# XuanHuang0/VANeRF

Hardware: AMD Instinct MI355X
Metric: rendered rays/sec (64 samples/ray) + PSNR vs ref, 512x334 view (higher is better)
Workload: dtype bf16x3 (bf16 MFMA on hi+lo split operands, f32 accumulate; per-sample outputs within 3.3e-5 of the f32 kernel); 1 GPU; configs/vanerf.json eval view 512x334, 64 coarse + 64 importance samples/ray, two-hand mesh 1558 verts / 3108 faces, 1 source view 256x256, random trained-like weights; rays=171008, parallelism=single

## Files before the change

include/vanerf_hip.h:

```cpp
#ifndef VANERF_HIP_H
#define VANERF_HIP_H

#include <stdint.h>

#ifdef __cplusplus
extern "C" {
#endif

#define VANERF_ABI_VERSION 12

#define VANERF_OK 0
#define VANERF_EINVAL (-22)
#define VANERF_ENOMEM (-12)
#define VANERF_EHIP (-5)

#define VANERF_NV 1558
#define VANERF_NV_HAND 779
#define VANERF_NKPT 42
#define VANERF_PE_LEVELS 3

typedef struct {
    const float* geo_at0_w1;
    const float* geo_at0_w2;
    const float* geo_ated0_w1;
// ... 73 lines not shown
    const float* sphere;
    const float* tnorm;
    const int32_t* orig;
    const float* cbox;
    int nfp, nc;
    const int32_t* cell_start;
    const int32_t* cell_tri;
    const float* cell_rec;
    const float* grid;
    const float* vsort;
    const float* vbox;
    int nvc;
    const float* cdisc;
} VanerfMeshAccel;

int64_t vanerf_mesh_accel_bytes(int nv, int nf, int G, int cell_capacity);
int vanerf_mesh_accel_build(const float* verts, int nv, const int32_t* faces, int nf, int G, int cell_capacity, void* tables,
                            int64_t tables_bytes, VanerfMeshAccel* out, void* stream);

int vanerf_mesh_query_accel(const VanerfMeshAccel* accel, const float* verts, int nv, const int32_t* faces, int nf,
                            const float* vert_vis, const float* pts, int64_t n, float* sdf, uint8_t* vis, int32_t* face,
                            int32_t* knn_idx, int grid_nx, int grid_ny, int grid_s, void* queue_word, void* stream);

int vanerf_knn1(const float* verts4, int nv, const float* pts, int64_t n, int32_t* idx, void* stream);

int vanerf_query_samples(const VanerfWeights* w, const VanerfFrame* frame, const float* pts, const float* query_sdf,
                         const uint8_t* query_vis, const int32_t* knn_idx, const float* noise, const int32_t* order, int raw, int64_t n,
                         float* out, uint8_t* valid, void* queue_word , const float* vertex_products,
                         void* stream);

int vanerf_vertex_products(const VanerfWeights* w, const VanerfFrame* frame, float* table, int64_t cap_floats, void* stream);

int vanerf_query_order(const VanerfFrame* frame, const float* pts, int64_t n, int32_t* order, void* scratch, int64_t scratch_bytes,
                       void* stream);
int64_t vanerf_query_order_scratch(int64_t n);

int vanerf_composite(const float* rgba, const float* z, const float* mesh_sdf, int Sa, const float* rgba_n, const float* mesh_sdf_n, int Sn,
                     const int32_t* src, int R, float beta, float* color, float* depth, float* alpha, float* sdf, float* contrib, void* stream);
int vanerf_composite_handle(const VanerfWeights* w, const float* rgba, const float* z, const float* mesh_sdf, int Sa, const float* rgba_n,
                            const float* mesh_sdf_n, int Sn, const int32_t* src, int R, float* color, float* depth, float* alpha, float* sdf,
                            float* contrib, void* stream);
int vanerf_eval_func(const float* raw_a, const uint8_t* valid_a, const float* raw_b, const uint8_t* valid_b, const int32_t* src, const float* noise,
                     int Sa, int Sb, int R, float invalid_sdf, float* rgba_a, float* rgba_b, void* stream);
int vanerf_composite_backward(const VanerfWeights* w, const float* rgba, const float* z, const float* mesh_sdf, int Sa, const float* rgba_n,
                              const float* mesh_sdf_n, int Sn, const int32_t* src, int R, const float* g_color, const float* g_depth,
                              const float* g_alpha, const float* g_sdf, float* d_rgba, float* d_rgba_n, float* d_beta, void* stream);
// ... 120 lines not shown
```

vanerf_amd/_ffi.py:

```python
import ctypes
import os

import torch
from ctypes import POINTER, Structure, c_char_p, c_double, c_float, c_int, c_int64, c_uint, c_uint64, c_void_p

_HERE = os.path.dirname(os.path.abspath(__file__))
LIB_PATH = os.environ.get("VANERF_HIP_LIB") or os.path.join(_HERE, "lib", "libvanerf_hip.so")
ABI_VERSION = 12
NUM_LAYERS = 20

if not os.path.exists(LIB_PATH):
    raise ImportError(f"{LIB_PATH} not found: the HIP extension is required (run `python -m vanerf_amd.build`)")
lib = ctypes.CDLL(LIB_PATH)

_FP = c_void_p


class VanerfWeightTable(Structure):
    _fields_ = [
        ("geo_at0_w1", _FP), ("geo_at0_w2", _FP), ("geo_ated0_w1", _FP), ("geo_ated0_w2", _FP),
        ("geo_at1_w1", _FP), ("geo_at1_w2", _FP), ("geo_ated1_w1", _FP), ("geo_ated1_w2", _FP),
        ("l1_v", _FP * 3), ("l1_g", _FP * 3), ("l1_b", _FP * 3), ("l1_w3", _FP), ("l1_b3", _FP),
        ("l2_v", _FP * 2), ("l2_g", _FP * 2), ("l2_b", _FP * 2), ("l2_w2", _FP), ("l2_b2", _FP),
        ("ibr_w", _FP), ("ibr_b", _FP),
# ... 34 lines not shown
    _fields_ = [("index", _FP), ("hit", _FP), ("z", _FP), ("color", _FP), ("depth", _FP), ("alpha", _FP), ("color_fine", _FP), ("depth_fine", _FP),
                ("alpha_fine", _FP), ("sdf", _FP), ("z_fine", _FP)]


_SIGS = {
    "vanerf_abi_version": (c_int, []),
    "vanerf_last_error": (c_char_p, []),
    "vanerf_mesh_cluster_size": (c_int, []),
    "vanerf_mesh_accel_bytes": (c_int64, [c_int, c_int, c_int, c_int]),
    "vanerf_mesh_accel_build": (c_int, [_FP, c_int, _FP, c_int, c_int, c_int, c_void_p, c_int64, POINTER(VanerfMeshAccel), c_void_p]),
    "vanerf_weights_pack": (c_int, [POINTER(VanerfWeightTable), c_int, POINTER(c_void_p)]),
    "vanerf_weights_free": (c_int, [c_void_p]),
    "vanerf_weights_update": (c_int, [c_void_p, POINTER(VanerfWeightTable), _FP, c_void_p]),
    "vanerf_weights_short_groups": (c_int, [c_void_p, POINTER(c_uint64)]),
    "vanerf_weights_pack_host": (c_int, [POINTER(VanerfWeightTable), _FP, c_int64, POINTER(c_int64), POINTER(c_uint)]),
    "vanerf_weights_stream_host": (c_int, [POINTER(VanerfWeightTable), c_int, _FP, c_int64, POINTER(c_int64)]),
    "vanerf_weights_download": (c_int, [c_void_p, c_int, _FP, c_int64, POINTER(c_int64)]),
    "vanerf_ray_setup": (c_int, [POINTER(VanerfPassDesc), _FP, _FP, _FP, _FP, _FP, _FP, _FP, c_void_p]),
    "vanerf_sample_points": (c_int, [_FP, _FP, _FP, c_int, c_int, c_int, _FP, c_void_p]),
    "vanerf_vertex_visibility": (c_int, [_FP, _FP, c_int, _FP, c_int, c_int, _FP, _FP, c_void_p]),
    "vanerf_mesh_query": (c_int, [_FP, c_int, _FP, c_int, _FP, _FP, c_int64, _FP, _FP, _FP, c_void_p]),
    "vanerf_mesh_query_accel": (c_int, [POINTER(VanerfMeshAccel), _FP, c_int, _FP, c_int, _FP, _FP, c_int64, _FP, _FP, _FP, _FP, c_int, c_int, c_int,
                                        _FP, c_void_p]),
    "vanerf_knn1": (c_int, [_FP, c_int, _FP, c_int64, _FP, c_void_p]),
    "vanerf_query_samples": (c_int, [c_void_p, POINTER(VanerfFrame), _FP, _FP, _FP, _FP, _FP, _FP, c_int, c_int64, _FP, _FP, _FP, _FP, c_void_p]),
    "vanerf_vertex_products": (c_int, [c_void_p, POINTER(VanerfFrame), _FP, c_int64, c_void_p]),
    "vanerf_query_forward_spill": (c_int, [c_void_p, POINTER(VanerfFrame), _FP, _FP, _FP, _FP, c_int64, c_int64, _FP, _FP, _FP, _FP, _FP, c_void_p]),
    "vanerf_query_backward": (c_int, [c_void_p, _FP, _FP, _FP, _FP, _FP, _FP, c_int64, c_int64, _FP, _FP, _FP, _FP, c_void_p]),
    "vanerf_weight_products": (c_int, [_FP, _FP, c_int64, c_int, c_int, _FP, c_void_p]),
    "vanerf_weight_products_size": (c_int, [POINTER(c_int64)]),
    "vanerf_spill_rows": (c_int, [POINTER(c_int), POINTER(c_int), POINTER(c_int), POINTER(c_int)]),
    "vanerf_layer_slots": (c_int, [c_int, _FP, c_int]),
    "vanerf_layer_rows": (c_int, [c_int, POINTER(c_int), POINTER(c_int), POINTER(c_int)]),
    "vanerf_query_order": (c_int, [POINTER(VanerfFrame), _FP, c_int64, _FP, _FP, c_int64, c_void_p]),
    "vanerf_query_order_scratch": (c_int64, [c_int64]),
    "vanerf_composite": (c_int, [_FP, _FP, _FP, c_int, _FP, _FP, c_int, _FP, c_int, c_float, _FP, _FP, _FP, _FP, _FP, c_void_p]),
    "vanerf_eval_func": (c_int, [_FP, _FP, _FP, _FP, _FP, _FP, c_int, c_int, c_int, c_float, _FP, _FP, c_void_p]),
    "vanerf_composite_handle": (c_int, [c_void_p, _FP, _FP, _FP, c_int, _FP, _FP, c_int, _FP, c_int, _FP, _FP, _FP, _FP, _FP, c_void_p]),
    "vanerf_composite_backward": (c_int, [c_void_p, _FP, _FP, _FP, c_int, _FP, _FP, c_int, _FP, c_int, _FP, _FP, _FP, _FP, _FP, _FP, _FP, c_void_p]),
    "vanerf_importance_merge": (c_int, [_FP, _FP, _FP, _FP, c_int, c_int, c_int, _FP, _FP, _FP, _FP, c_void_p]),
    "vanerf_importance_sample": (c_int, [_FP, _FP, _FP, _FP, c_int, c_int, c_int, _FP, _FP, c_void_p]),
    "vanerf_render_pass_scratch": (c_int64, [c_int, c_int, c_int, c_int, c_int, c_int]),
    "vanerf_render_pass": (c_int, [c_void_p, POINTER(VanerfFrame), POINTER(VanerfMeshAccel), _FP, c_int, _FP, c_int, POINTER(VanerfPassDesc),
                                   POINTER(VanerfPassOut), _FP, c_int64, _FP, c_void_p]),
    "vanerf_scatter_add_rows": (c_int, [_FP, _FP, _FP, c_int64, c_int64, c_int, _FP, c_int, c_void_p]),
    "vanerf_bilinear_taps": (c_int, [_FP, c_int64, c_int, c_int, _FP, _FP, c_void_p]),
# ... 46 lines not shown
```

vanerf_amd/csrc/mesh_kernels.hip:

```cpp
#include "common.h"

using namespace vanerf;

namespace {

struct f3 { float x, y, z; };
__device__ __forceinline__ f3 sub3(f3 a, f3 b) { return {a.x - b.x, a.y - b.y, a.z - b.z}; }
__device__ __forceinline__ float dot3(f3 a, f3 b) { return (a.x * b.x + a.y * b.y) + a.z * b.z; }
__device__ __forceinline__ f3 madd3(f3 a, f3 d, float t) { return {a.x + d.x * t, a.y + d.y * t, a.z + d.z * t}; }

__device__ __forceinline__ float point_tri_dist2_q(f3 p, f3 a, f3 b, f3 c, f3& q)
{
    const f3 ab = sub3(b, a), ac = sub3(c, a), ap = sub3(p, a);
    const float d1 = dot3(ab, ap), d2 = dot3(ac, ap);
    if (d1 <= 0.0f && d2 <= 0.0f) {
        q = a;
    } else {
        const f3 bp = sub3(p, b);
        const float d3 = dot3(ab, bp), d4 = dot3(ac, bp);
        if (d3 >= 0.0f && d4 <= d3) {
            q = b;
        } else {
            const float vc = d1 * d4 - d3 * d2;
            if (vc <= 0.0f && d1 >= 0.0f && d3 <= 0.0f) {
// ... 281 lines not shown
    v = OP(v, DPP<0x142, 0xA>(v));                                                                        \
    v = OP(v, DPP<0x143, 0xC>(v));
__device__ __forceinline__ float wave_min_f(float v) { VANERF_WAVE_REDUCE(float, dpp_f, fminf) return __int_as_float(__builtin_amdgcn_readlane(__float_as_int(v), 63)); }
__device__ __forceinline__ float wave_max_f(float v) { VANERF_WAVE_REDUCE(float, dpp_f, fmaxf) return __int_as_float(__builtin_amdgcn_readlane(__float_as_int(v), 63)); }
__device__ __forceinline__ int wave_min_i(int v) { VANERF_WAVE_REDUCE(int, dpp_i, min) return __builtin_amdgcn_readlane(v, 63); }
#undef VANERF_WAVE_REDUCE

__device__ __forceinline__ float uni(float v) { return __int_as_float(__builtin_amdgcn_readfirstlane(__float_as_int(v))); }

__device__ __forceinline__ float box_dist2(f3 p, const float* b)
{
    const float dx = fmaxf(fmaxf(b[0] - p.x, p.x - b[3]), 0.0f);
    const float dy = fmaxf(fmaxf(b[1] - p.y, p.y - b[4]), 0.0f);
    const float dz = fmaxf(fmaxf(b[2] - p.z, p.z - b[5]), 0.0f);
    return (dx * dx + dy * dy) + dz * dz;
}

template <int ND>
__global__ __launch_bounds__(MA_BLOCK) void mesh_query_accel_kernel(const VanerfMeshAccel A, const float* __restrict__ V,
                                                                    const int32_t* __restrict__ F, const float* __restrict__ vert_vis,
                                                                    const float* __restrict__ P, long long n, float* __restrict__ sdf,
                                                                    uint8_t* __restrict__ vis, int32_t* __restrict__ face,
                                                                    int32_t* __restrict__ knn, int gnx, int gny, int gS,
                                                                    unsigned long long* __restrict__ queue)
{
    extern __shared__ float4 s_dyn[];
    __shared__ unsigned short s_list[MA_BLOCK / 64][TL_LIST];
    __shared__ __attribute__((aligned(16))) float s_cand[MA_BLOCK / 64][TL_CAND][12];
    __shared__ float s_dit[MA_BLOCK / 64][TL_IT][64];
    float4* s_vs = s_dyn;
    float* s_vbox = reinterpret_cast<float*>(s_vs + A.nvc * CL);
    float* s_box = s_vbox + A.nvc * 6;
    for (int k = threadIdx.x; k < A.nc * 6; k += MA_BLOCK) s_box[k] = A.cbox[k];
    for (int k = threadIdx.x; k < A.nvc * 6; k += MA_BLOCK) s_vbox[k] = A.vbox[k];
    for (int k = threadIdx.x; k < A.nvc * CL; k += MA_BLOCK) s_vs[k] = reinterpret_cast<const float4*>(A.vsort)[k];
    const float grid_y0 = A.grid[0], grid_z0 = A.grid[1], grid_cy = A.grid[2], grid_cz = A.grid[3];
    const int grid_G = __float_as_int(A.grid[4]);
    __syncthreads();
    const int lane = threadIdx.x & 63;
    auto lane_now = [&]() { int l = lane; asm volatile("" : "+v"(l)); return l; };
    auto claim = [&]() {
        unsigned long long v = 0ull;
        if (lane == 0) v = atomicAdd(queue, 1ull);
        return (long long)(((unsigned long long)(unsigned)__builtin_amdgcn_readfirstlane((int)(v >> 32)) << 32) |
                           (unsigned)__builtin_amdgcn_readfirstlane((int)v));
    };
    const int ntx = (gnx + 7) >> 3, nty = (gny + 7) >> 3;
    const int gD = (gS + ND - 1) / ND;
    const long long nwork = gnx > 0 ? (long long)ntx * nty * gD : (n + 64 * ND - 1) / (64 * ND);
#ifdef VANERF_MESH_PHASES
    unsigned long long ph[16] = {}, tprev = __builtin_amdgcn_s_memtime();
#endif
    for (long long w = claim(); w < nwork; w = claim()) {
        int item_d0 = 0, item_x0 = 0, item_y0 = 0;
        if (gnx > 0) {
            const unsigned wu = (unsigned)w, tile = wu / (unsigned)gD;
            item_d0 = __builtin_amdgcn_readfirstlane((int)(wu % (unsigned)gD) * ND);
            item_x0 = __builtin_amdgcn_readfirstlane((int)(tile % (unsigned)ntx) * 8);
            item_y0 = __builtin_amdgcn_readfirstlane((int)(tile / (unsigned)ntx) * 8);
        }
        auto locate = [&](int k, bool& act) -> long long {
            long long i;
            if (gnx > 0) {
                const int d = item_d0 + k;
                const int l = lane_now();
                const int rx = item_x0 + (l & 7), ry = item_y0 + (l >> 3);
                act = rx < gnx && ry < gny && d < gS;
                i = ((long long)min(ry, gny - 1) * gnx + min(rx, gnx - 1)) * gS + min(d, gS - 1);
            } else {
                i = (w * ND + k) * 64 + lane;
                act = i < n;
                i = act ? i : n - 1;
            }
            return i;
        };
        f3 pk[ND];
#pragma unroll
        for (int k = 0; k < ND; ++k) {
            bool act;
            const long long i = locate(k, act);
            pk[k] = {P[3 * i], P[3 * i + 1], P[3 * i + 2]};
        }
        MPH(0);
        float tlo[3] = {pk[0].x, pk[0].y, pk[0].z}, thi[3] = {pk[0].x, pk[0].y, pk[0].z};
#pragma unroll
        for (int k = 1; k < ND; ++k) {
// ... 592 lines not shown
        if (n == 0) return;
        if (!verts || !faces || !vert_vis || !pts || !sdf || !vis) throw_error("vanerf_mesh_query: null argument");
        if (nv <= 0 || nf <= 0 || n < 0) throw_error("vanerf_mesh_query: nv=%d nf=%d n=%lld", nv, nf, (long long)n);
        if (n == 0) return;
        hipLaunchKernelGGL(mesh_query_kernel, dim3((unsigned)((n + MQ_BLOCK - 1) / MQ_BLOCK)), dim3(MQ_BLOCK), 0, (hipStream_t)stream,
                           verts, faces, nf, vert_vis, pts, (long long)n, sdf, vis, face);
        HIP_CHECK(hipGetLastError());
    });
}

extern "C" int vanerf_knn1(const float* verts4, int nv, const float* pts, int64_t n, int32_t* idx, void* stream)
{
    return guarded([&] {
        if (n == 0) return;
        if (!verts4 || !pts || !idx) throw_error("vanerf_knn1: null argument");
        if (nv <= 0 || nv > 8192 || n < 0) throw_error("vanerf_knn1: nv=%d n=%lld", nv, (long long)n);
        if (n == 0) return;
        hipLaunchKernelGGL(knn1_kernel, dim3((unsigned)((n + 255) / 256)), dim3(256), sizeof(float4) * nv, (hipStream_t)stream,
                           reinterpret_cast<const float4*>(verts4), nv, pts, (long long)n, idx);
        HIP_CHECK(hipGetLastError());
    });
}

extern "C" int vanerf_mesh_query_accel(const VanerfMeshAccel* accel, const float* verts, int nv, const int32_t* faces, int nf,
                                       const float* vert_vis, const float* pts, int64_t n, float* sdf, uint8_t* vis, int32_t* face,
                                       int32_t* knn_idx, int grid_nx, int grid_ny, int grid_s, void* queue_word, void* stream)
{
    return guarded([&] {
        if (n == 0) return;
        if (!accel || !verts || !faces || !vert_vis || !pts || !sdf || !vis) throw_error("vanerf_mesh_query_accel: null argument");
        const VanerfMeshAccel& A = *accel;
        if (!A.tri || !A.sphere || !A.tnorm || !A.orig || !A.cbox || !A.cdisc || !A.cell_start || !A.cell_tri || !A.cell_rec || !A.grid) throw_error("vanerf_mesh_query_accel: accel has a null pointer");
        if (A.nc <= 0 || A.nc > MA_MAX_CLUSTERS || A.nfp != A.nc * CL || A.nfp < nf) throw_error("vanerf_mesh_query_accel: bad cluster table (nc=%d nfp=%d nf=%d)", A.nc, A.nfp, nf);
        if (nv <= 0 || nf <= 0 || n < 0) throw_error("vanerf_mesh_query_accel: nv=%d nf=%d n=%lld", nv, nf, (long long)n);
        if (!A.vsort || !A.vbox || A.nvc <= 0 || A.nvc > MA_MAX_VCLUSTERS || A.nvc * CL < nv)
            throw_error("vanerf_mesh_query_accel: bad vertex cluster table (nvc=%d nv=%d)", A.nvc, nv);
        const size_t lds = sizeof(float) * ((size_t)A.nvc * CL * 4 + (size_t)A.nvc * 6 + (size_t)A.nc * 6);
        if (lds > 140 * 1024) throw_error("vanerf_mesh_query_accel: mesh too large for the LDS-resident tables (%zu bytes)", lds);
        if (lds > 64 * 1024) {
            HIP_CHECK(hipFuncSetAttribute(reinterpret_cast<const void*>(mesh_query_accel_kernel<1>), hipFuncAttributeMaxDynamicSharedMemorySize, (int)lds));
            HIP_CHECK(hipFuncSetAttribute(reinterpret_cast<const void*>(mesh_query_accel_kernel<ND_MAX>), hipFuncAttributeMaxDynamicSharedMemorySize, (int)lds));
        }
        if (n == 0) return;
        if (grid_nx != 0 && (grid_nx < 0 || grid_ny <= 0 || grid_s <= 0 || (long long)grid_nx * grid_ny * grid_s != n))
            throw_error("vanerf_mesh_query_accel: ray-grid hint %d x %d x %d does not match n = %lld", grid_nx, grid_ny, grid_s, (long long)n);
        if (n >= (1ll << 36)) throw_error("vanerf_mesh_query_accel: n = %lld points in one launch (limit 2^36)", (long long)n);
        if (!queue_word || (reinterpret_cast<uintptr_t>(queue_word) & 7u)) throw_error("vanerf_mesh_query_accel: queue_word must be 8 bytes of device memory, 8-byte aligned");
        struct PerDevice { std::atomic<size_t> lds{~(size_t)0}; std::atomic<int> resident{0}; };
        static PerDevice per_device[64];
        int dev = 0;
        HIP_CHECK(hipGetDevice(&dev));
        PerDevice& pd = per_device[dev & 63];
        if (pd.resident.load() == 0 || pd.lds.load() != lds) {
            int cus = 256, per_cu = 1;
            HIP_CHECK(hipDeviceGetAttribute(&cus, hipDeviceAttributeMultiprocessorCount, dev));
            HIP_CHECK(hipOccupancyMaxActiveBlocksPerMultiprocessor(&per_cu, mesh_query_accel_kernel<ND_MAX>, MA_BLOCK, lds));
            pd.resident.store(cus * (per_cu > 0 ? per_cu : 1));
            pd.lds.store(lds);
        }
        const int resident = pd.resident.load();
        unsigned long long* const queue = static_cast<unsigned long long*>(queue_word);
        HIP_CHECK(hipMemsetAsync(queue, 0, sizeof(unsigned long long), (hipStream_t)stream));
        long long blocks = (n + MA_BLOCK - 1) / MA_BLOCK;
        if (blocks > resident) blocks = resident;
        const long long waves = (long long)resident * (MA_BLOCK / 64), items_nd = (n + 64 * ND_MAX - 1) / (64 * ND_MAX);
        if (ND_MAX > 1 && items_nd >= 4 * waves)
            hipLaunchKernelGGL(mesh_query_accel_kernel<ND_MAX>, dim3((unsigned)blocks), dim3(MA_BLOCK), lds, (hipStream_t)stream, A, verts, faces, vert_vis,
                               pts, (long long)n, sdf, vis, face, knn_idx, grid_nx, grid_ny, grid_s, queue);
        else
            hipLaunchKernelGGL(mesh_query_accel_kernel<1>, dim3((unsigned)blocks), dim3(MA_BLOCK), lds, (hipStream_t)stream, A, verts, faces, vert_vis,
                               pts, (long long)n, sdf, vis, face, knn_idx, grid_nx, grid_ny, grid_s, queue);
        HIP_CHECK(hipGetLastError());
    });
}

#ifdef VANERF_MESH_PHASES
extern "C" int vanerf_debug_mesh_phases(unsigned long long* out8, int reset)
{
    return guarded([&] {
        HIP_CHECK(hipMemcpyFromSymbol(out8, HIP_SYMBOL(g_ma_phase), sizeof(unsigned long long) * 16));
        if (reset) { unsigned long long z[16] = {}; HIP_CHECK(hipMemcpyToSymbol(HIP_SYMBOL(g_ma_phase), z, sizeof z)); }
    });
}
#endif

extern "C" int vanerf_mesh_cluster_size(void) { return CL; }

namespace {

constexpr int AB_THREADS = 1024;

__device__ __forceinline__ unsigned part1by2(unsigned x)
{
    x = (x | (x << 16)) & 0x030000FFu;
    x = (x | (x << 8)) & 0x0300F00Fu;
    x = (x | (x << 4)) & 0x030C30C3u;
    return (x | (x << 2)) & 0x09249249u;
}

__device__ __forceinline__ unsigned morton30(f3 c, f3 lo, f3 hi)
{
    auto q = [](float v, float l, float h) { return (unsigned)fminf(fmaxf((v - l) / (h - l + 1e-9f) * 1023.0f, 0.0f), 1023.0f); };
    return part1by2(q(c.x, lo.x, hi.x)) | (part1by2(q(c.y, lo.y, hi.y)) << 1) | (part1by2(q(c.z, lo.z, hi.z)) << 2);
}

__device__ __forceinline__ f3 vert3(const float* V, int i) { return {V[3 * i], V[3 * i + 1], V[3 * i + 2]}; }

__device__ void bitonic_sort_lds(unsigned long long* s, int n)
{
// ... 378 lines not shown
```

vanerf_amd/csrc/pass.cpp:

```cpp
#include "common.h"

using namespace vanerf;

namespace {

constexpr int64_t ALIGN = 256;
constexpr int64_t PARTITION_MIN_SAMPLES = 1 << 18;

struct Carver {
    char* base;
    int64_t off = 0;
    explicit Carver(void* b) : base(static_cast<char*>(b)) {}
    template <class T> T* take(int64_t n)
    {
        T* p = base ? reinterpret_cast<T*>(base + off) : nullptr;
        off += ((n * (int64_t)sizeof(T) + ALIGN - 1) / ALIGN) * ALIGN;
        return p;
    }
};

struct Layout {
    float *rays_d, *cam_pos, *near, *far, *pts, *q_sdf_c, *rgba_c, *contrib, *z_new, *q_sdf_f, *rgba_f, *z_fine, *color_f3, *s1;
    float *raw_c, *rgba_cf;
    uint8_t *valid_c, *valid_f;
    uint8_t *q_vis;
    int32_t *knn, *order, *src;
    unsigned long long* queue_words;
    void* order_scratch;
    int64_t order_scratch_bytes, total;
};

Layout carve(void* base, int R, int Sc, int Sf, int fine, int reuse, int n_views)
{
    Carver c(base);
    Layout L{};
    const int64_t nc = (int64_t)R * Sc, nf = fine ? (int64_t)R * (reuse ? Sf : Sc + Sf) : 0, nmax = nc > nf ? nc : nf;
    L.queue_words = c.take<unsigned long long>(4);
    L.rays_d = c.take<float>(3LL * R);
    L.cam_pos = c.take<float>(4LL * n_views);
    L.near = c.take<float>(R);
    L.far = c.take<float>(R);
    L.pts = c.take<float>(3 * nmax);
    L.q_vis = c.take<uint8_t>(nmax);
    L.knn = c.take<int32_t>(nmax);
    L.order = c.take<int32_t>(nmax);
    L.order_scratch_bytes = vanerf_query_order_scratch(nmax);
    L.order_scratch = c.take<uint8_t>(L.order_scratch_bytes);
    L.q_sdf_c = c.take<float>(nc);
    L.rgba_c = c.take<float>(5 * nc);
    L.contrib = c.take<float>(nc);
    if (fine) {
        L.z_new = c.take<float>((int64_t)R * Sf);
        L.src = c.take<int32_t>((int64_t)R * (Sc + Sf));
        L.z_fine = c.take<float>((int64_t)R * (Sc + Sf));
        L.q_sdf_f = c.take<float>(nf);
        L.rgba_f = c.take<float>(5 * nf);
        if (reuse == 2) {
            L.raw_c = c.take<float>(5 * nc);
            L.rgba_cf = c.take<float>(5 * nc);
            L.valid_c = c.take<uint8_t>(nc);
            L.valid_f = c.take<uint8_t>(nf);
        }
    }
    L.color_f3 = c.take<float>(3LL * R);
    L.s1 = c.take<float>(4LL * R);
    L.total = c.off;
    return L;
}

void ok(int rc, const char* what)
{
    if (rc != VANERF_OK) {
        const std::string inner = vanerf_last_error();
        throw Error(rc, std::string("vanerf_render_pass: ") + what + ": " + inner);
    }
}

void run_marches(const VanerfWeights* w, const VanerfFrame* frame, const VanerfMeshAccel* accel, const float* verts, int nv, const int32_t* faces, int nf,
                 const VanerfPassDesc& d, int reuse, const float* vertex_products, const Layout& L, const VanerfPassOut& o, void* stream)
{
    const int R = d.n_views * d.nx * d.ny, Sc = d.Sc, Sf = d.Sf;
    const int rays_per_view = d.cams ? d.nx * d.ny : 0;
    const int grid_nx = d.pixels_xy ? 0 : d.nx, grid_ny = d.pixels_xy ? 0 : d.n_views * d.ny;
    int marches = 0;
    auto march = [&](const float* z, int S, const float* noise, float* q_sdf, float* rgba, uint8_t* valid_raw = nullptr) {
        unsigned long long* const qw = L.queue_words + 2 * marches++;
        const int64_t n = (int64_t)R * S;
        ok(vanerf_sample_points(L.rays_d, L.cam_pos, z, R, rays_per_view, S, L.pts, stream), "sample points");
        ok(vanerf_mesh_query_accel(accel, verts, nv, faces, nf, frame->vert_vis, L.pts, n, q_sdf, L.q_vis, nullptr, L.knn, grid_nx, grid_ny, grid_nx ? S : 0, qw,
                                   stream), "mesh query");
        const int32_t* order = nullptr;
        if (n >= PARTITION_MIN_SAMPLES) {
            ok(vanerf_query_order(frame, L.pts, n, L.order, L.order_scratch, L.order_scratch_bytes, stream), "validity partition");
            order = L.order;
        }
        ok(vanerf_query_samples(w, frame, L.pts, q_sdf, L.q_vis, L.knn, noise, order, valid_raw ? 1 : 0, n, rgba, valid_raw, qw + 1, vertex_products, stream),
           "per-sample networks");
    };
    if (reuse == 2) {
        march(o.z, Sc, nullptr, L.q_sdf_c, L.raw_c, L.valid_c);
        ok(vanerf_eval_func(L.raw_c, L.valid_c, nullptr, nullptr, nullptr, d.noise_c, Sc, 0, R, frame->invalid_sdf, L.rgba_c, nullptr, stream), "eval_func (coarse)");
    } else {
        march(o.z, Sc, d.noise_c, L.q_sdf_c, L.rgba_c);
    }
    ok(vanerf_composite_handle(w, L.rgba_c, o.z, L.q_sdf_c, Sc, nullptr, nullptr, 0, nullptr, R, o.color, o.depth, o.alpha, L.s1, L.contrib, stream), "composite");
    if (!d.fine) return;
    float* z_fine = o.z_fine ? o.z_fine : L.z_fine;
    float* cf = o.color_fine ? o.color_fine : L.color_f3;
    float* df = o.depth_fine ? o.depth_fine : L.s1 + R;
    float* af = o.alpha_fine ? o.alpha_fine : L.s1 + 2LL * R;
    float* sf = o.sdf ? o.sdf : L.s1 + 3LL * R;
    ok(vanerf_importance_merge(L.contrib, o.z, d.u, d.u ? nullptr : d.t_lin_f, R, Sc, Sf, L.z_new, z_fine, L.src, nullptr, stream), "importance sampling");
    if (reuse == 2) {
// ... 52 lines not shown
```

vanerf_amd/renderer.py:

```python
import ctypes
import dataclasses
import os
import weakref
from ctypes import byref, c_float, c_int64, c_uint, c_void_p

import torch
import torch.nn.functional as F

from . import _ffi
from ._ffi import VanerfFrame, VanerfMeshAccel, VanerfPassDesc, VanerfPassOut, VanerfWeightTable, check, lib

NV, NV_HAND, NKPT = 1558, 779, 42


def _ptr(t, dtype=None, cuda=True):
    if t is None:
        return None
    if dtype is not None and t.dtype != dtype:
        raise TypeError(f"expected {dtype}, got {t.dtype}")
    if cuda and not t.is_cuda:
        raise ValueError("the HIP render path needs device tensors (no CPU fallback)")
    if not t.is_contiguous():
        raise ValueError("tensor must be contiguous")
    return c_void_p(t.data_ptr())
# ... 391 lines not shown
    vis = torch.empty(H, W, dtype=f32, device=dev)
    p2f = torch.empty(H, W, dtype=torch.int32, device=dev) if want_raster else None
    zbuf = torch.empty(H, W, dtype=f32, device=dev) if want_raster else None
    check(lib.vanerf_render_vis(_ptr(verts3, f32), nv, _ptr(faces_i32, torch.int32), faces_i32.shape[0], _ptr(vert_vis, f32), _ptr(R, f32),
                                _ptr(T, f32), _ptr(focal, f32), _ptr(princpt, f32), int(H), int(W), _ptr(scratch), scratch.numel() * 4, _ptr(rgb),
                                _ptr(vis), _ptr(p2f), _ptr(zbuf), _stream()))
    return (rgb, vis, p2f, zbuf) if want_raster else (rgb, vis)


def mesh_query(verts3, faces_i32, vert_vis, pts, want_face=False):
    n = pts.shape[0]
    sdf = torch.empty(n, dtype=torch.float32, device=pts.device)
    vis = torch.empty(n, dtype=torch.uint8, device=pts.device)
    face = torch.empty(n, dtype=torch.int32, device=pts.device) if want_face else None
    check(lib.vanerf_mesh_query(_ptr(verts3, torch.float32), verts3.shape[0], _ptr(faces_i32, torch.int32), faces_i32.shape[0],
                                _ptr(vert_vis, torch.float32), _ptr(pts, torch.float32), n, _ptr(sdf), _ptr(vis), _ptr(face), _stream()))
    return (sdf, vis, face) if want_face else (sdf, vis)


def _queue_word(dev):
    return torch.empty(2, dtype=torch.int32, device=dev)


def mesh_query_accel(accel, verts3, faces_i32, vert_vis, pts, want_face=False, want_knn=True, grid=None):
    gnx, gny, gs = grid if grid is not None else (0, 0, 0)
    n = pts.shape[0]
    sdf = torch.empty(n, dtype=torch.float32, device=pts.device)
    vis = torch.empty(n, dtype=torch.uint8, device=pts.device)
    face = torch.empty(n, dtype=torch.int32, device=pts.device) if want_face else None
    knn = torch.empty(n, dtype=torch.int32, device=pts.device) if want_knn else None
    check(lib.vanerf_mesh_query_accel(byref(accel.c), _ptr(verts3, torch.float32), verts3.shape[0], _ptr(faces_i32, torch.int32),
                                      faces_i32.shape[0], _ptr(vert_vis, torch.float32), _ptr(pts, torch.float32), n, _ptr(sdf), _ptr(vis),
                                      _ptr(face), _ptr(knn), int(gnx), int(gny), int(gs), _ptr(_queue_word(pts.device)), _stream()))
    return tuple(t for t in (sdf, vis, face, knn) if t is not None)


def knn1(verts4, pts):
    idx = torch.empty(pts.shape[0], dtype=torch.int32, device=pts.device)
    check(lib.vanerf_knn1(_ptr(verts4, torch.float32), verts4.shape[0], _ptr(pts, torch.float32), pts.shape[0], _ptr(idx), _stream()))
    return idx


def query_order(frame, pts):
    n = pts.shape[0]
    order = torch.empty(n, dtype=torch.int32, device=pts.device)
    nbytes = int(lib.vanerf_query_order_scratch(n))
    scratch = torch.empty(nbytes, dtype=torch.uint8, device=pts.device)
    check(lib.vanerf_query_order(byref(frame.c), _ptr(pts, torch.float32), n, _ptr(order, torch.int32), _ptr(scratch, torch.uint8), nbytes, _stream()))
    return order


def query_samples(weights, frame, pts, query_sdf, query_vis, knn_idx, noise=None, want_valid=False, raw=False, order=None, vertex_products="auto"):
    vp = frame.vertex_products(weights) if isinstance(vertex_products, str) else vertex_products
    n = pts.shape[0]
    out = torch.empty(n, 5, dtype=torch.float32, device=pts.device)
    valid = torch.empty(n, dtype=torch.uint8, device=pts.device) if want_valid else None
# ... 245 lines not shown
        for k in ("rays_d", "cam_pos", "z"):
            if k in inject:
                if inject[k].shape != rays[k].shape or inject[k].dtype != torch.float32:
                    raise ValueError(f"inject[{k!r}] must be float32 of shape {tuple(rays[k].shape)}")
                rays[k] = inject[k].contiguous()
    if inject is not None and "z_fine" in inject:
        reuse_coarse = False
    noisy_reuse = noise_std > 0.0 and fine and reuse_coarse
    if noise_draws is not None and (noise_draws[0].numel() != R * Sc or (fine and noise_draws[1].numel() != R * (Sc + Sf))):
        raise ValueError("noise_draws: one draw per evaluated sample (R*Sc coarse, R*(Sc+Sf) fine)")

    def scaled(draws, n):
        dev = frame.verts3.device
        draws = torch.randn(n, device=dev, generator=generator) if draws is None else draws.reshape(-1).to(dev, torch.float32)
        return (draws * noise_std).contiguous()

    def eval_func(raw, valid, noise):
        n = raw.shape[0]
        out = torch.empty(n, 5, dtype=torch.float32, device=raw.device)
        check(lib.vanerf_eval_func(_ptr(raw, torch.float32), _ptr(valid, torch.uint8), None, None, None, _ptr(noise, torch.float32), 1, 0, n,
                                   float(frame.c.invalid_sdf), _ptr(out), None, _stream()))
        return out

    def evaluate(z, draws=None, raw=False):
        pts = sample_points(rays["rays_d"], rays["cam_pos"], z)
        grid = (nx, ny, z.shape[1]) if pixels is None else None
        q_sdf, q_vis, knn = mesh_query_accel(frame.accel, frame.verts3, frame.faces, frame.vert_vis, pts, grid=grid)
        noise = scaled(draws, pts.shape[0]) if noise_std > 0.0 and not raw else None
        order = query_order(frame, pts) if pts.shape[0] >= PARTITION_MIN_SAMPLES else None
        if kernel_events is not None:
            e0, e1 = torch.cuda.Event(enable_timing=True), torch.cuda.Event(enable_timing=True)
            e0.record()
        res = query_samples(weights, frame, pts, q_sdf, q_vis, knn, noise, order=order, raw=raw, want_valid=raw)
        if kernel_events is not None:
            e1.record()
            kernel_events.append((e0, e1, pts.shape[0]))
        d = dict(pts=pts, q_sdf=q_sdf.view(R, -1), q_vis=q_vis, knn=knn, noise=noise)
        if raw:
            d["raw"], d["valid"] = res
        else:
            d["rgba"] = res.view(R, -1, 5)
        return d

    if noisy_reuse:
        c = evaluate(rays["z"], raw=True)
        c["noise"] = scaled(None if noise_draws is None else noise_draws[0], R * Sc)
        c["rgba"] = eval_func(c["raw"], c["valid"], c["noise"]).view(R, Sc, 5)
    else:
        c = evaluate(rays["z"], None if noise_draws is None else noise_draws[0])
    c["color"], c["depth"], c["alpha"], c["contrib"], c["sdf"] = composite(c["rgba"], rays["z"], c["q_sdf"], weights)
    out = {"color": c["color"], "depth": c["depth"], "alpha": c["alpha"], "index": rays["index"], "z": rays["z"], "hit": rays["hit"],
           "rays_d": rays["rays_d"], "cam_pos": rays["cam_pos"]}
    if debug:
        out["coarse"] = c
    if fine:
        if inject is not None and "z_fine" in inject:
            z_new, z_fine, src = None, inject["z_fine"].contiguous(), None
            if z_fine.shape != (R, Sc + Sf):
                raise ValueError("inject['z_fine'] must have shape (R, Sc + Sf)")
        else:
            z_new, z_fine, src = importance_merge(c["contrib"], rays["z"], Sf, u=u)
        cf = None
        if noisy_reuse:
            ids = torch.where(src >= 0, src, Sc + (-src - 1)).long()
            pos = torch.empty_like(ids).scatter_(1, ids, torch.arange(Sc + Sf, device=ids.device).expand(R, -1))
            noise_f = scaled(None if noise_draws is None else noise_draws[1], R * (Sc + Sf)).view(R, Sc + Sf)
            f = evaluate(z_new, raw=True)
            f["noise"] = noise_f.gather(1, pos[:, Sc:]).reshape(-1).contiguous()
            f["rgba"] = eval_func(f["raw"], f["valid"], f["noise"]).view(R, Sf, 5)
            cf = {"noise": noise_f.gather(1, pos[:, :Sc]).reshape(-1).contiguous()}
            cf["rgba"] = eval_func(c["raw"], c["valid"], cf["noise"]).view(R, Sc, 5)
            f["color"], f["depth"], f["alpha"], f["contrib"], f["sdf"] = composite_merged(cf["rgba"], c["q_sdf"], f["rgba"], f["q_sdf"], src,
                                                                                          z_fine, weights, want_contrib=debug)
        elif reuse_coarse:
            f = evaluate(z_new)
            f["color"], f["depth"], f["alpha"], f["contrib"], f["sdf"] = composite_merged(c["rgba"], c["q_sdf"], f["rgba"], f["q_sdf"], src,
                                                                                          z_fine, weights, want_contrib=debug)
        else:
            f = evaluate(z_fine, None if noise_draws is None else noise_draws[1])
            f["color"], f["depth"], f["alpha"], f["contrib"], f["sdf"] = composite(f["rgba"], z_fine, f["q_sdf"], weights, want_contrib=debug)
        out.update({"color_fine": f["color"], "depth_fine": f["depth"], "alpha_fine": f["alpha"], "sdf": f["sdf"], "z_fine": z_fine, "z_new": z_new})
        if debug:
            out["fine"] = f
            out["fine_src"] = src if reuse_coarse else None
            out["coarse_in_fine"] = cf
    return out


def _pass_outputs(lead, Sc, Sf, fine, dev):
    def new(*tail, dtype=torch.float32):
        return torch.empty(*lead, *tail, dtype=dtype, device=dev)

    out = {"index": new(dtype=torch.int64), "hit": new(dtype=torch.uint8), "z": new(Sc), "color": new(3), "depth": new(), "alpha": new()}
    if fine:
        out.update({"color_fine": new(3), "depth_fine": new(), "alpha_fine": new(), "sdf": new(), "z_fine": new(Sc + Sf)})
    o = VanerfPassOut()
    for k, _ in VanerfPassOut._fields_:
        setattr(o, k, _ptr(out.get(k)))
    return out, o


def _run_pass(weights, frame, d, scratch=None):
# ... 83 lines not shown
```

Before: 11.72 million rays/s.

## Sort samples by depth within 8x8 pixel tiles before mesh query

Adds a kernel that merge-sorts, in LDS, all samples of each 8x8 pixel tile by their z value and writes a per-tile permutation. The mesh query kernel can take this order, so each wave processes samples at similar depths. That should make traversal of the spatial grid and triangle cells more coherent and cut divergence. It costs an extra sort launch and buffer per march plus an indirect index load. It is enabled by default for both coarse and fine marches through an environment knob.

```diff
diff --git a/include/vanerf_hip.h b/include/vanerf_hip.h
--- a/include/vanerf_hip.h
+++ b/include/vanerf_hip.h
@@ -119,6 +119,12 @@
                             const float* vert_vis, const float* pts, int64_t n, float* sdf, uint8_t* vis, int32_t* face,
                             int32_t* knn_idx, int grid_nx, int grid_ny, int grid_s, void* queue_word, void* stream);
 
+int vanerf_mesh_query_accel_ordered(const VanerfMeshAccel* accel, const float* verts, int nv, const int32_t* faces, int nf,
+                                    const float* vert_vis, const float* pts, int64_t n, float* sdf, uint8_t* vis, int32_t* face,
+                                    int32_t* knn_idx, int grid_nx, int grid_ny, int grid_s, void* queue_word, const int32_t* item_order,
+                                    void* stream);
+int vanerf_mesh_tile_order(const float* z, int grid_nx, int grid_ny, int grid_s, int32_t* order, void* stream);
+
 int vanerf_knn1(const float* verts4, int nv, const float* pts, int64_t n, int32_t* idx, void* stream);
 
 int vanerf_query_samples(const VanerfWeights* w, const VanerfFrame* frame, const float* pts, const float* query_sdf,
diff --git a/vanerf_amd/_ffi.py b/vanerf_amd/_ffi.py
--- a/vanerf_amd/_ffi.py
+++ b/vanerf_amd/_ffi.py
@@ -80,6 +80,9 @@
     "vanerf_mesh_query": (c_int, [_FP, c_int, _FP, c_int, _FP, _FP, c_int64, _FP, _FP, _FP, c_void_p]),
     "vanerf_mesh_query_accel": (c_int, [POINTER(VanerfMeshAccel), _FP, c_int, _FP, c_int, _FP, _FP, c_int64, _FP, _FP, _FP, _FP, c_int, c_int, c_int,
                                         _FP, c_void_p]),
+    "vanerf_mesh_query_accel_ordered": (c_int, [POINTER(VanerfMeshAccel), _FP, c_int, _FP, c_int, _FP, _FP, c_int64, _FP, _FP, _FP, _FP, c_int, c_int,
+                                                c_int, _FP, _FP, c_void_p]),
+    "vanerf_mesh_tile_order": (c_int, [_FP, c_int, c_int, c_int, _FP, c_void_p]),
     "vanerf_knn1": (c_int, [_FP, c_int, _FP, c_int64, _FP, c_void_p]),
     "vanerf_query_samples": (c_int, [c_void_p, POINTER(VanerfFrame), _FP, _FP, _FP, _FP, _FP, _FP, c_int, c_int64, _FP, _FP, _FP, _FP, c_void_p]),
     "vanerf_vertex_products": (c_int, [c_void_p, POINTER(VanerfFrame), _FP, c_int64, c_void_p]),
diff --git a/vanerf_amd/csrc/mesh_kernels.hip b/vanerf_amd/csrc/mesh_kernels.hip
--- a/vanerf_amd/csrc/mesh_kernels.hip
+++ b/vanerf_amd/csrc/mesh_kernels.hip
@@ -327,7 +327,8 @@
                                                                     const float* __restrict__ P, long long n, float* __restrict__ sdf,
                                                                     uint8_t* __restrict__ vis, int32_t* __restrict__ face,
                                                                     int32_t* __restrict__ knn, int gnx, int gny, int gS,
-                                                                    unsigned long long* __restrict__ queue)
+                                                                    unsigned long long* __restrict__ queue,
+                                                                    const int32_t* __restrict__ item_order)
 {
     extern __shared__ float4 s_dyn[];
     __shared__ unsigned short s_list[MA_BLOCK / 64][TL_LIST];
@@ -357,16 +358,25 @@
     unsigned long long ph[16] = {}, tprev = __builtin_amdgcn_s_memtime();
 #endif
     for (long long w = claim(); w < nwork; w = claim()) {
-        int item_d0 = 0, item_x0 = 0, item_y0 = 0;
+        int item_d0 = 0, item_x0 = 0, item_y0 = 0, item_tile = 0;
         if (gnx > 0) {
             const unsigned wu = (unsigned)w, tile = wu / (unsigned)gD;
+            item_tile = __builtin_amdgcn_readfirstlane((int)tile);
             item_d0 = __builtin_amdgcn_readfirstlane((int)(wu % (unsigned)gD) * ND);
             item_x0 = __builtin_amdgcn_readfirstlane((int)(tile % (unsigned)ntx) * 8);
             item_y0 = __builtin_amdgcn_readfirstlane((int)(tile / (unsigned)ntx) * 8);
         }
         auto locate = [&](int k, bool& act) -> long long {
             long long i;
-            if (gnx > 0) {
+            if (gnx > 0 && item_order) {
+                const int d = item_d0 + k;
+                int idx = item_order[((long long)item_tile * gS + min(d, gS - 1)) * 64 + lane_now()];
+                const bool named = (unsigned long long)(unsigned)idx < (unsigned long long)n;
+                const unsigned long long m = __ballot(named);
+                const int first = __builtin_amdgcn_readlane(idx, m ? __builtin_ctzll(m) : 0);
+                act = named && d < gS;
+                i = named ? idx : m ? first : 0;
+            } else if (gnx > 0) {
                 const int d = item_d0 + k;
                 const int l = lane_now();
                 const int rx = item_x0 + (l & 7), ry = item_y0 + (l >> 3);
@@ -1005,12 +1015,15 @@
     });
 }
 
-extern "C" int vanerf_mesh_query_accel(const VanerfMeshAccel* accel, const float* verts, int nv, const int32_t* faces, int nf,
-                                       const float* vert_vis, const float* pts, int64_t n, float* sdf, uint8_t* vis, int32_t* face,
-                                       int32_t* knn_idx, int grid_nx, int grid_ny, int grid_s, void* queue_word, void* stream)
+extern "C" int vanerf_mesh_query_accel_ordered(const VanerfMeshAccel* accel, const float* verts, int nv, const int32_t* faces, int nf,
+                                               const float* vert_vis, const float* pts, int64_t n, float* sdf, uint8_t* vis, int32_t* face,
+                                               int32_t* knn_idx, int grid_nx, int grid_ny, int grid_s, void* queue_word,
+                                               const int32_t* item_order, void* stream)
 {
     return guarded([&] {
         if (n == 0) return;
+        if (item_order && grid_nx <= 0) throw_error("vanerf_mesh_query_accel_ordered: an item order needs the ray-grid hint");
+        if (item_order && n > 0x7fffffffLL) throw_error("vanerf_mesh_query_accel_ordered: n = %lld does not fit the table's 32-bit sample indices", (long long)n);
         if (!accel || !verts || !faces || !vert_vis || !pts || !sdf || !vis) throw_error("vanerf_mesh_query_accel: null argument");
         const VanerfMeshAccel& A = *accel;
         if (!A.tri || !A.sphere || !A.tnorm || !A.orig || !A.cbox || !A.cdisc || !A.cell_start || !A.cell_tri || !A.cell_rec || !A.grid) throw_error("vanerf_mesh_query_accel: accel has a null pointer");
@@ -1049,12 +1062,20 @@
         const long long waves = (long long)resident * (MA_BLOCK / 64), items_nd = (n + 64 * ND_MAX - 1) / (64 * ND_MAX);
         if (ND_MAX > 1 && items_nd >= 4 * waves)
             hipLaunchKernelGGL(mesh_query_accel_kernel<ND_MAX>, dim3((unsigned)blocks), dim3(MA_BLOCK), lds, (hipStream_t)stream, A, verts, faces, vert_vis,
-                               pts, (long long)n, sdf, vis, face, knn_idx, grid_nx, grid_ny, grid_s, queue);
+                               pts, (long long)n, sdf, vis, face, knn_idx, grid_nx, grid_ny, grid_s, queue, item_order);
         else
             hipLaunchKernelGGL(mesh_query_accel_kernel<1>, dim3((unsigned)blocks), dim3(MA_BLOCK), lds, (hipStream_t)stream, A, verts, faces, vert_vis,
-                               pts, (long long)n, sdf, vis, face, knn_idx, grid_nx, grid_ny, grid_s, queue);
+                               pts, (long long)n, sdf, vis, face, knn_idx, grid_nx, grid_ny, grid_s, queue, item_order);
         HIP_CHECK(hipGetLastError());
     });
+}
+
+extern "C" int vanerf_mesh_query_accel(const VanerfMeshAccel* accel, const float* verts, int nv, const int32_t* faces, int nf,
+                                       const float* vert_vis, const float* pts, int64_t n, float* sdf, uint8_t* vis, int32_t* face,
+                                       int32_t* knn_idx, int grid_nx, int grid_ny, int grid_s, void* queue_word, void* stream)
+{
+    return vanerf_mesh_query_accel_ordered(accel, verts, nv, faces, nf, vert_vis, pts, n, sdf, vis, face, knn_idx, grid_nx, grid_ny, grid_s, queue_word,
+                                           nullptr, stream);
 }
 
 #ifdef VANERF_MESH_PHASES
@@ -1068,6 +1089,106 @@
 #endif
 
 extern "C" int vanerf_mesh_cluster_size(void) { return CL; }
+
+namespace {
+
+constexpr int TO_BLOCK = 1024;
+constexpr int TO_MAX_S = 128;
+static_assert(64 * TO_MAX_S <= 65536, "the index within a tile is kept in 16 bits");
+
+__global__ __launch_bounds__(TO_BLOCK) void mesh_tile_order_kernel(const float* __restrict__ z, int gnx, int gny, int S, int32_t* __restrict__ order)
+{
+    extern __shared__ unsigned s_tile[];
+    const int N = 64 * S;
+    unsigned* src = s_tile;
+    unsigned* dst = s_tile + N;
+    unsigned short* src_i = reinterpret_cast<unsigned short*>(s_tile + 2 * N);
+    unsigned short* dst_i = src_i + N;
+    const int ntx = (gnx + 7) >> 3;
+    const int x0 = (int)(blockIdx.x % (unsigned)ntx) * 8, y0 = (int)(blockIdx.x / (unsigned)ntx) * 8;
+    for (int e = threadIdx.x; e < N; e += TO_BLOCK) {
+        const int l = e / S, d = e - l * S;
+        const int rx = x0 + (l & 7), ry = y0 + (l >> 3);
+        unsigned u = 0xffffffffu;
+        if (rx < gnx && ry < gny) {
+            u = __float_as_uint(z[((long long)ry * gnx + rx) * S + d] + 0.0f);
+            u ^= (u >> 31) ? 0xffffffffu : 0x80000000u;
+            u = min(u, 0xfffffffeu);
+        }
+        src[e] = u;
+        src_i[e] = (unsigned short)e;
+    }
+    __syncthreads();
+    int descends = 0;
+    for (int e = threadIdx.x; e < N; e += TO_BLOCK) descends |= (e % S != 0) && src[e - 1] > src[e];
+    for (int L = __syncthreads_or(descends) ? 1 : S; L < N; L *= 2) {
+        const int E = (L & 3) ? 1 : 4;
+        for (int c = threadIdx.x * E; c < N; c += TO_BLOCK * E) {
+            unsigned key4[4] = {};
+            unsigned idx4[4] = {};
+            if (E == 4) {
+                const uint4 k = *reinterpret_cast<const uint4*>(src + c);
+                const uint2 i = *reinterpret_cast<const uint2*>(src_i + c);
+                key4[0] = k.x; key4[1] = k.y; key4[2] = k.z; key4[3] = k.w;
+                idx4[0] = i.x & 0xffffu; idx4[1] = i.x >> 16; idx4[2] = i.y & 0xffffu; idx4[3] = i.y >> 16;
+            } else {
+                key4[0] = src[c];
+                idx4[0] = src_i[c];
+            }
+            const int a0 = c / (2 * L) * (2 * L), b0 = min(a0 + L, N), end = min(a0 + 2 * L, N);
+            const bool in_a = c < b0;
+            const unsigned* const sib = src + (in_a ? b0 : a0);
+            const int len = in_a ? end - b0 : L;
+            const int place0 = c - b0 + (in_a ? b0 : a0);
+            int lo = 0;
+#pragma unroll
+            for (int j = 0; j < 4; ++j) {
+                if (j >= E) break;
+                const unsigned key = key4[j];
+                auto below = [&](int i) { return in_a ? sib[i] < key : sib[i] <= key; };
+                int hi = len;
+                if (j > 0) {
+                    for (int step = 1; lo + step - 1 < hi; step *= 2) {
+                        const int p = lo + step - 1;
+                        if (below(p)) lo = p + 1; else { hi = p; break; }
+                    }
+                }
+                while (lo < hi) {
+                    const int mid = (lo + hi) >> 1;
+                    if (below(mid)) lo = mid + 1; else hi = mid;
+                }
+                dst[place0 + j + lo] = key;
+                dst_i[place0 + j + lo] = (unsigned short)idx4[j];
+            }
+        }
+        __syncthreads();
+        unsigned* const t = src; src = dst; dst = t;
+        unsigned short* const ti = src_i; src_i = dst_i; dst_i = ti;
+    }
+    for (int e = threadIdx.x; e < N; e += TO_BLOCK) {
+        const int local = src_i[e], l = local / S, d = local - l * S;
+        const int rx = x0 + (l & 7), ry = y0 + (l >> 3);
+        order[(long long)blockIdx.x * N + e] = (rx < gnx && ry < gny) ? (ry * gnx + rx) * S + d : -1;
+    }
+}
+
+}
+
+extern "C" int vanerf_mesh_tile_order(const float* z, int grid_nx, int grid_ny, int grid_s, int32_t* order, void* stream)
+{
+    return guarded([&] {
+        if (!z || !order) throw_error("vanerf_mesh_tile_order: null argument");
+        if (grid_nx <= 0 || grid_ny <= 0 || grid_s <= 0) throw_error("vanerf_mesh_tile_order: grid %d x %d x %d", grid_nx, grid_ny, grid_s);
+        if (grid_s > TO_MAX_S) throw_error("vanerf_mesh_tile_order: %d samples per ray (limit %d: a tile is sorted in LDS)", grid_s, TO_MAX_S);
+        const long long tiles = (long long)((grid_nx + 7) >> 3) * ((grid_ny + 7) >> 3);
+        if (tiles * 64 * grid_s > 0x7fffffffLL) throw_error("vanerf_mesh_tile_order: grid %d x %d x %d does not fit 32-bit sample indices", grid_nx, grid_ny, grid_s);
+        const size_t lds = (sizeof(unsigned) + sizeof(unsigned short)) * 2 * 64 * (size_t)grid_s;
+        if (lds > 64 * 1024)
+            HIP_CHECK(hipFuncSetAttribute(reinterpret_cast<const void*>(mesh_tile_order_kernel), hipFuncAttributeMaxDynamicSharedMemorySize, (int)lds));
+        hipLaunchKernelGGL(mesh_tile_order_kernel, dim3((unsigned)tiles), dim3(TO_BLOCK), lds, (hipStream_t)stream, z, grid_nx, grid_ny, grid_s, order);
+        HIP_CHECK(hipGetLastError());
+    });
+}
 
 namespace {
 
diff --git a/vanerf_amd/csrc/pass.cpp b/vanerf_amd/csrc/pass.cpp
--- a/vanerf_amd/csrc/pass.cpp
+++ b/vanerf_amd/csrc/pass.cpp
@@ -1,4 +1,6 @@
 #include "common.h"
+
+#include <cstdlib>
 
 using namespace vanerf;
 
@@ -24,7 +26,8 @@
     float *raw_c, *rgba_cf;
     uint8_t *valid_c, *valid_f;
     uint8_t *q_vis;
-    int32_t *knn, *order, *src;
+    int32_t *knn, *order, *src, *tile_order;
+    int64_t tile_order_slots;
     unsigned long long* queue_words;
     void* order_scratch;
     int64_t order_scratch_bytes, total;
@@ -46,6 +49,8 @@
     L.order = c.take<int32_t>(nmax);
     L.order_scratch_bytes = vanerf_query_order_scratch(nmax);
     L.order_scratch = c.take<uint8_t>(L.order_scratch_bytes);
+    L.tile_order_slots = (5 * nmax + 3) / 4;
+    L.tile_order = c.take<int32_t>(L.tile_order_slots);
     L.q_sdf_c = c.take<float>(nc);
     L.rgba_c = c.take<float>(5 * nc);
     L.contrib = c.take<float>(nc);
@@ -68,6 +73,15 @@
     return L;
 }
 
+constexpr int MESH_TILE_ORDER_MAX_S = 128;
+constexpr int MESH_TILE_ORDER_DEFAULT = 3;
+
+int mesh_tile_order_mode()
+{
+    const char* e = std::getenv("VANERF_MESH_TILE_ORDER");
+    return (e && e[0] >= '0' && e[0] <= '3' && !e[1]) ? e[0] - '0' : MESH_TILE_ORDER_DEFAULT;
+}
+
 void ok(int rc, const char* what)
 {
     if (rc != VANERF_OK) {
@@ -83,12 +97,20 @@
     const int rays_per_view = d.cams ? d.nx * d.ny : 0;
     const int grid_nx = d.pixels_xy ? 0 : d.nx, grid_ny = d.pixels_xy ? 0 : d.n_views * d.ny;
     int marches = 0;
+    const int tile_order_mode = mesh_tile_order_mode();
     auto march = [&](const float* z, int S, const float* noise, float* q_sdf, float* rgba, uint8_t* valid_raw = nullptr) {
+        const bool fine_launch = marches > 0;
         unsigned long long* const qw = L.queue_words + 2 * marches++;
         const int64_t n = (int64_t)R * S;
         ok(vanerf_sample_points(L.rays_d, L.cam_pos, z, R, rays_per_view, S, L.pts, stream), "sample points");
-        ok(vanerf_mesh_query_accel(accel, verts, nv, faces, nf, frame->vert_vis, L.pts, n, q_sdf, L.q_vis, nullptr, L.knn, grid_nx, grid_ny, grid_nx ? S : 0, qw,
-                                   stream), "mesh query");
+        const int32_t* tile_order = nullptr;
+        const int64_t slots = (int64_t)((grid_nx + 7) / 8) * ((grid_ny + 7) / 8) * 64 * S;
+        if (grid_nx && S <= MESH_TILE_ORDER_MAX_S && slots <= L.tile_order_slots && (tile_order_mode & (fine_launch ? 2 : 1))) {
+            ok(vanerf_mesh_tile_order(z, grid_nx, grid_ny, S, L.tile_order, stream), "mesh tile order");
+            tile_order = L.tile_order;
+        }
+        ok(vanerf_mesh_query_accel_ordered(accel, verts, nv, faces, nf, frame->vert_vis, L.pts, n, q_sdf, L.q_vis, nullptr, L.knn, grid_nx, grid_ny,
+                                           grid_nx ? S : 0, qw, tile_order, stream), "mesh query");
         const int32_t* order = nullptr;
         if (n >= PARTITION_MIN_SAMPLES) {
             ok(vanerf_query_order(frame, L.pts, n, L.order, L.order_scratch, L.order_scratch_bytes, stream), "validity partition");
diff --git a/vanerf_amd/renderer.py b/vanerf_amd/renderer.py
--- a/vanerf_amd/renderer.py
+++ b/vanerf_amd/renderer.py
@@ -437,16 +437,37 @@
     return torch.empty(2, dtype=torch.int32, device=dev)
 
 
-def mesh_query_accel(accel, verts3, faces_i32, vert_vis, pts, want_face=False, want_knn=True, grid=None):
+MESH_TILE_ORDER_MAX_S = 128
+MESH_TILE_ORDER_DEFAULT = 3
+
+
+def mesh_tile_order_mode():
+    e = os.environ.get("VANERF_MESH_TILE_ORDER", "")
+    return int(e) if e in ("0", "1", "2", "3") else MESH_TILE_ORDER_DEFAULT
+
+
+def mesh_tile_order(z, nx, ny):
+    S = z.shape[1]
+    if z.shape[0] != nx * ny:
+        raise ValueError(f"mesh_tile_order: {z.shape[0]} rays for a {nx} x {ny} grid")
+    order = torch.empty(((nx + 7) // 8) * ((ny + 7) // 8), S, 64, dtype=torch.int32, device=z.device)
+    check(lib.vanerf_mesh_tile_order(_ptr(z, torch.float32), int(nx), int(ny), int(S), _ptr(order), _stream()))
+    return order
+
+
+def mesh_query_accel(accel, verts3, faces_i32, vert_vis, pts, want_face=False, want_knn=True, grid=None, item_order=None):
     gnx, gny, gs = grid if grid is not None else (0, 0, 0)
+    if item_order is not None and item_order.numel() != ((gnx + 7) // 8) * ((gny + 7) // 8) * 64 * gs:
+        raise ValueError("mesh_query_accel: item_order does not have 64 * S slots per 8 x 8 pixel tile of the grid")
     n = pts.shape[0]
     sdf = torch.empty(n, dtype=torch.float32, device=pts.device)
     vis = torch.empty(n, dtype=torch.uint8, device=pts.device)
     face = torch.empty(n, dtype=torch.int32, device=pts.device) if want_face else None
     knn = torch.empty(n, dtype=torch.int32, device=pts.device) if want_knn else None
-    check(lib.vanerf_mesh_query_accel(byref(accel.c), _ptr(verts3, torch.float32), verts3.shape[0], _ptr(faces_i32, torch.int32),
-                                      faces_i32.shape[0], _ptr(vert_vis, torch.float32), _ptr(pts, torch.float32), n, _ptr(sdf), _ptr(vis),
-                                      _ptr(face), _ptr(knn), int(gnx), int(gny), int(gs), _ptr(_queue_word(pts.device)), _stream()))
+    check(lib.vanerf_mesh_query_accel_ordered(byref(accel.c), _ptr(verts3, torch.float32), verts3.shape[0], _ptr(faces_i32, torch.int32),
+                                              faces_i32.shape[0], _ptr(vert_vis, torch.float32), _ptr(pts, torch.float32), n, _ptr(sdf), _ptr(vis),
+                                              _ptr(face), _ptr(knn), int(gnx), int(gny), int(gs), _ptr(_queue_word(pts.device)),
+                                              _ptr(item_order, torch.int32), _stream()))
     return tuple(t for t in (sdf, vis, face, knn) if t is not None)
 
 
@@ -738,10 +759,14 @@
                                    float(frame.c.invalid_sdf), _ptr(out), None, _stream()))
         return out
 
-    def evaluate(z, draws=None, raw=False):
+    tile_order_mode = mesh_tile_order_mode()
+
+    def evaluate(z, draws=None, raw=False, fine_launch=False):
         pts = sample_points(rays["rays_d"], rays["cam_pos"], z)
         grid = (nx, ny, z.shape[1]) if pixels is None else None
-        q_sdf, q_vis, knn = mesh_query_accel(frame.accel, frame.verts3, frame.faces, frame.vert_vis, pts, grid=grid)
+        use_order = grid is not None and z.shape[1] <= MESH_TILE_ORDER_MAX_S and tile_order_mode & (2 if fine_launch else 1)
+        item_order = mesh_tile_order(z, nx, ny) if use_order else None
+        q_sdf, q_vis, knn = mesh_query_accel(frame.accel, frame.verts3, frame.faces, frame.vert_vis, pts, grid=grid, item_order=item_order)
         noise = scaled(draws, pts.shape[0]) if noise_std > 0.0 and not raw else None
         order = query_order(frame, pts) if pts.shape[0] >= PARTITION_MIN_SAMPLES else None
         if kernel_events is not None:
@@ -781,7 +806,7 @@
             ids = torch.where(src >= 0, src, Sc + (-src - 1)).long()
             pos = torch.empty_like(ids).scatter_(1, ids, torch.arange(Sc + Sf, device=ids.device).expand(R, -1))
             noise_f = scaled(None if noise_draws is None else noise_draws[1], R * (Sc + Sf)).view(R, Sc + Sf)
-            f = evaluate(z_new, raw=True)
+            f = evaluate(z_new, raw=True, fine_launch=True)
             f["noise"] = noise_f.gather(1, pos[:, Sc:]).reshape(-1).contiguous()
             f["rgba"] = eval_func(f["raw"], f["valid"], f["noise"]).view(R, Sf, 5)
             cf = {"noise": noise_f.gather(1, pos[:, :Sc]).reshape(-1).contiguous()}
@@ -789,11 +814,11 @@
             f["color"], f["depth"], f["alpha"], f["contrib"], f["sdf"] = composite_merged(cf["rgba"], c["q_sdf"], f["rgba"], f["q_sdf"], src,
                                                                                           z_fine, weights, want_contrib=debug)
         elif reuse_coarse:
-            f = evaluate(z_new)
+            f = evaluate(z_new, fine_launch=True)
             f["color"], f["depth"], f["alpha"], f["contrib"], f["sdf"] = composite_merged(c["rgba"], c["q_sdf"], f["rgba"], f["q_sdf"], src,
                                                                                           z_fine, weights, want_contrib=debug)
         else:
-            f = evaluate(z_fine, None if noise_draws is None else noise_draws[1])
+            f = evaluate(z_fine, None if noise_draws is None else noise_draws[1], fine_launch=True)
             f["color"], f["depth"], f["alpha"], f["contrib"], f["sdf"] = composite(f["rgba"], z_fine, f["q_sdf"], weights, want_contrib=debug)
         out.update({"color_fine": f["color"], "depth_fine": f["depth"], "alpha_fine": f["alpha"], "sdf": f["sdf"], "z_fine": z_fine, "z_new": z_new})
         if debug:
```

Measured after the change: 12.11 million rays/s (median of 6 runs). +3.4%, better.
